# praateekmahajan/moving-mnist-vae

Hardware: AMD Instinct MI355X
Metric: frames/sec/GPU VAE train step, 20×64×64 batch; ELBO vs CPU ref (higher is better)
Workload: dtype bf16; 1 GPU; BASELINE configs[1]: 256 clips x 20 frames x 64x64 per GPU per step (=5120 frames), conv-VAE z=128, Gaussian NLL sigma=0.1 + KL (normal_vae_1_kl_0_mmd), Adam, random-init weights, Bernoulli(0.0521) q=2 labels; parallelism=dp1, rccl_ranks=1, grad_exchange=none, bn=per-rank batch statistics

## Files before the change

moving-mnist-vae_amd/csrc/conv_deep2.inc:

```
#include "kernels.hpp"
#include "tile_common.hpp"

namespace mmvae {

template <typename T, typename TO, int NPT, int CPT, bool ACC, bool LITE, bool F8 = false>
__device__ __forceinline__ void deep2_conv_body(const DeepArgs& a) {
  static_assert(!F8 || (sizeof(T) == 2 && !ACC), "fp8 MFMA: bf16 storage, forward convolutions");
  constexpr int VE = Elem<T>::kVec;
  constexpr int ES = sizeof(T);
  constexpr int TPX = NPT * 16;
  constexpr int kSV = 8;
  constexpr int G = CPT < (LITE ? 2 : 4) ? CPT : (LITE ? 2 : 4);
  constexpr int NB = LITE ? 2 : NPT >= 8 ? 3 : 4;
  constexpr int UPT = CPT / G;
  extern __shared__ __attribute__((aligned(16))) char smem[];
  const int t = threadIdx.x, nthr = blockDim.x, lane = t & 63, wv = __builtin_amdgcn_readfirstlane(t >> 6), gq = lane >> 4, r = lane & 15;
  const int c0 = (blockIdx.y * a.nw + wv) * 32;
  const int cin_vecs = a.Cin / VE;
  constexpr int LES = F8 ? 1 : ES;
  const int pitch = F8 ? a.Cin + 16 : a.Cin * ES + 32;
  const int npix_in = a.ipt * a.Hi * a.Wi;
  char* sPatch = smem;
  unsigned* sOpix = reinterpret_cast<unsigned*>(sPatch + (size_t)(npix_in + 1) * pitch);
  float* sStat = reinterpret_cast<float*>(sOpix + TPX) + wv * 64;
  unsigned short* sTab = reinterpret_cast<unsigned short*>(sOpix + TPX + 64 * a.nw);
  const T* __restrict__ X = reinterpret_cast<const T*>(a.x);
  TO* __restrict__ Y = reinterpret_cast<TO*>(a.y);
  const bool has_pro = a.pro_scale != nullptr, has_bias = a.bias != nullptr, has_stats = a.stats != nullptr;
  const float relu_lo = a.pro_relu ? 0.f : -__builtin_inff();
  const int HqWq = a.Hq * a.Wq;

  const int cv = t % cin_vecs, pix0 = t / cin_vecs, PS = nthr / cin_vecs;
  for (int p = t; p < TPX; p += nthr) {
    unsigned o = ~0u;
    int img = 0, hq = 0, wq = 0;
    const bool live = p < a.ipt * HqWq;
    if (live) {
      img = p / HqWq;
      const int rem = p - img * HqWq;
      hq = rem / a.Wq; wq = rem - hq * a.Wq;
      o = ((unsigned)img << 16) | ((unsigned)hq << 8) | (unsigned)wq;
    }
    sOpix[p] = o;
    const int hb = hq * a.SI, wb = wq * a.SI, ib = img * a.Hi;
#pragma unroll
    for (int tap = 0; tap < kMaxTaps; ++tap)
      if (tap < a.ntaps_all) {
        const int hi = hb + a.taps[tap].dh, wi = wb + a.taps[tap].dw;
        const bool in = live && hi >= 0 && hi < a.Hi && wi >= 0 && wi < a.Wi;
        sTab[tap * TPX + p] = (unsigned short)(in ? (ib + hi) * a.Wi + wi : npix_in);
      }
  }
  for (int i = t; i < pitch / 16; i += nthr) reinterpret_cast<Vec16*>(sPatch + (size_t)npix_in * pitch)[i] = Vec16{{0, 0, 0, 0}};
  sStat[lane] = 0.f;

  for (int tile = blockIdx.x; tile < a.ntiles; tile += gridDim.x) {
    const int n0 = tile * a.ipt;
    const int nimg = min(a.ipt, a.N - n0);
    __syncthreads();
    {
      const T* src = X + (long)n0 * a.Hi * a.Wi * a.Cin + cv * VE;
      const int nvalid = nimg * a.Hi * a.Wi;
      float psc[VE], psh[VE];
#pragma unroll
      for (int j = 0; j < VE; j += 4) {
        const float4 sc = has_pro ? *reinterpret_cast<const float4*>(a.pro_scale + cv * VE + j) : make_float4(1.f, 1.f, 1.f, 1.f);
        const float4 sh = has_pro ? *reinterpret_cast<const float4*>(a.pro_shift + cv * VE + j) : make_float4(0.f, 0.f, 0.f, 0.f);
        psc[j] = sc.x; psc[j + 1] = sc.y; psc[j + 2] = sc.z; psc[j + 3] = sc.w;
        psh[j] = sh.x; psh[j + 1] = sh.y; psh[j + 2] = sh.z; psh[j + 3] = sh.w;
      }
      for (int p0 = pix0; p0 < npix_in; p0 += kSV * PS) {
        Vec16 q[kSV];
#pragma unroll
        for (int k = 0; k < kSV; ++k) {
          const int p = p0 + k * PS;
          q[k] = Vec16{{0, 0, 0, 0}};
          if (p < nvalid) q[k] = *reinterpret_cast<const Vec16*>(src + (long)p * a.Cin);
        }
#pragma unroll
        for (int k = 0; k < kSV; ++k) {
          const int p = p0 + k * PS;
          if (p < npix_in) {
            if (has_pro && p < nvalid) {
              float f[VE];
              Elem<T>::unpack(q[k], f);
#pragma unroll
              for (int j = 0; j < VE; ++j) f[j] = fmaxf(f[j] * psc[j] + psh[j], relu_lo);
              q[k] = Elem<T>::pack(f);
            }
            if constexpr (F8) {
              float f[VE];
              Elem<T>::unpack(q[k], f);
              *reinterpret_cast<uint2*>(sPatch + (size_t)p * pitch + cv * 8) = pack8_fp8(f);
            } else {
              *reinterpret_cast<Vec16*>(sPatch + (size_t)p * pitch + cv * 16) = q[k];
            }
          }
        }
      }
    }
    __syncthreads();
    for (int ph = 0; ph < a.nphase; ++ph) {
      const DeepPhase P = a.phases[ph];
      const long rowbytes = (long)P.ntaps * a.Cin * LES;
      const int cstride = a.wfrag ? 1024 : 64;
      const char* wl0 = reinterpret_cast<const char*>(a.w) + P.w_off * LES +
                        (a.wfrag ? (long)c0 * rowbytes + lane * 16 : (long)(c0 + 8 * (r >> 2) + (r & 3)) * rowbytes + gq * 16);
      const char* wl1 = wl0 + (a.wfrag ? 16 : 4) * rowbytes;
      f32x4 acc[2][NPT];
#pragma unroll
      for (int m = 0; m < 2; ++m)
#pragma unroll
        for (int pt = 0; pt < NPT; ++pt) acc[m][pt] = (f32x4){0, 0, 0, 0};
      const int nunits = P.ntaps * UPT;
      auto load_unit = [&](Vec16 (&buf)[G][2], int unit) {
        const int jb = min(unit, nunits - 1) * G * cstride;
#pragma unroll
        for (int g = 0; g < G; ++g) {
          buf[g][0] = *reinterpret_cast<const Vec16*>(wl0 + jb + g * cstride);
          buf[g][1] = *reinterpret_cast<const Vec16*>(wl1 + jb + g * cstride);
        }
      };
      auto tap_pixels = [&](unsigned (&pb)[NPT], int tap) {
        const unsigned short* tb = sTab + (P.tap0 + tap) * TPX + r;
#pragma unroll
        for (int pt = 0; pt < NPT; ++pt) pb[pt] = __umul24((unsigned)tb[pt * 16], (unsigned)pitch) + gq * (F8 ? 8 : 16);
      };
      auto mul_unit = [&](const Vec16 (&buf)[G][2], const unsigned (&pb)[NPT], int cc0) {
#pragma unroll
        for (int g = 0; g < G; ++g) {
          if constexpr (F8) {
            long bl[NPT], bh[NPT];
#pragma unroll
            for (int pt = 0; pt < NPT; ++pt) {
              bl[pt] = *reinterpret_cast<const long*>(sPatch + pb[pt] + (cc0 + g) * 64);
              bh[pt] = *reinterpret_cast<const long*>(sPatch + pb[pt] + (cc0 + g) * 64 + 32);
            }
#pragma unroll
            for (int m = 0; m < 2; ++m) {
              const long al = (long)(((unsigned long)buf[g][m].w[1] << 32) | buf[g][m].w[0]);
              const long ah = (long)(((unsigned long)buf[g][m].w[3] << 32) | buf[g][m].w[2]);
#pragma unroll
              for (int pt = 0; pt < NPT; ++pt) {
                acc[m][pt] = __builtin_amdgcn_mfma_f32_16x16x32_fp8_fp8(al, bl[pt], acc[m][pt], 0, 0, 0);
                acc[m][pt] = __builtin_amdgcn_mfma_f32_16x16x32_fp8_fp8(ah, bh[pt], acc[m][pt], 0, 0, 0);
              }
            }
          } else {
            Vec16 bf[NPT];
#pragma unroll
            for (int pt = 0; pt < NPT; ++pt) bf[pt] = *reinterpret_cast<const Vec16*>(sPatch + pb[pt] + (cc0 + g) * 64);
#pragma unroll
            for (int pt = 0; pt < NPT; ++pt) {
              acc[0][pt] = mma_vec<T>(buf[g][0], bf[pt], acc[0][pt]);
              acc[1][pt] = mma_vec<T>(buf[g][1], bf[pt], acc[1][pt]);
            }
          }
        }
      };
      Vec16 buf[NB][G][2];
      unsigned pb[NPT];
#pragma unroll
      for (int b = 0; b < NB - 1; ++b) load_unit(buf[b], b);
      for (int u = 0; u < nunits; u += NB) {
#pragma unroll
        for (int b = 0; b < NB; ++b) {
          const int uu = u + b;
          load_unit(buf[(b + NB - 1) % NB], uu + NB - 1);
          __builtin_amdgcn_sched_barrier(0);
          if (uu < nunits) {
            if (UPT == 1 || (uu & (UPT - 1)) == 0) tap_pixels(pb, uu / UPT);
            mul_unit(buf[b], pb, (uu & (UPT - 1)) * G);
          }
          __builtin_amdgcn_sched_barrier(0);
        }
      }
      float bv[8], st1[8], st2[8];
#pragma unroll
      for (int j = 0; j < 8; ++j) {
        bv[j] = has_bias ? a.bias[c0 + 8 * gq + j] : 0.f;
        st1[j] = 0.f; st2[j] = 0.f;
      }
#pragma unroll
      for (int pt = 0; pt < NPT; ++pt) {
        const unsigned op = sOpix[pt * 16 + r];
        const int img = (int)(op >> 16), hq = (int)((op >> 8) & 255u), wq = (int)(op & 255u);
        if (op != ~0u && img < nimg && hq < P.Hq && wq < P.Wq) {
          const unsigned ob = ((((unsigned)(n0 + img) * a.Ho + (unsigned)(hq * a.SO + P.ph)) * a.Wo + (unsigned)(wq * a.SO + P.pw)) * (unsigned)a.Cout) +
                              (unsigned)(c0 + 8 * gq);
          float v[8];
#pragma unroll
          for (int j = 0; j < 8; ++j) v[j] = acc[j >> 2][pt][j & 3] + bv[j];
#pragma unroll
          for (int j = 0; j < 8; ++j) { st1[j] += v[j]; st2[j] += v[j] * v[j]; }
          dstore8<TO>(Y + ob, v, ACC);
        }
      }
      if (has_stats) {
#pragma unroll
        for (int j = 0; j < 8; ++j) { st1[j] = row16_sum(st1[j]); st2[j] = row16_sum(st2[j]); }
        if (r == 0) {
#pragma unroll
          for (int j = 0; j < 8; ++j) {
            sStat[8 * gq + j] += st1[j];
            sStat[32 + 8 * gq + j] += st2[j];
          }
        }
      }
    }
  }
  if (has_stats) {
    a.stats[(long)blockIdx.x * 2 * a.Cout + (long)(lane >> 5) * a.Cout + c0 + (lane & 31)] = sStat[lane];
  }
}

template <typename T, typename TO, int NPT, int CPT, bool ACC>
__global__ __launch_bounds__(512, 2) void deep2_conv_kernel(DeepArgs a) { deep2_conv_body<T, TO, NPT, CPT, ACC, false>(a); }
template <typename T, typename TO, int NPT, int CPT, bool ACC>
__global__ __launch_bounds__(512, 3) void deep2_conv_lite_kernel(DeepArgs a) { deep2_conv_body<T, TO, NPT, CPT, ACC, true>(a); }
template <typename T, typename TO, int NPT, int CPT, bool ACC>
__global__ __launch_bounds__(512, 2) void deep2_conv_f8_kernel(DeepArgs a) { deep2_conv_body<T, TO, NPT, CPT, false, false, true>(a); }
template <typename T, typename TO, int NPT, int CPT, bool ACC>
__global__ __launch_bounds__(512, 3) void deep2_conv_f8_lite_kernel(DeepArgs a) { deep2_conv_body<T, TO, NPT, CPT, false, true, true>(a); }

template <typename T, typename TO>
static int launch_deep2_t(const DeepArgs& a, int dt, int gx, hipStream_t s) {
  const size_t lds = deep2_conv_lds_bytes(a, dt);
  dim3 grid(gx, a.Cout / (32 * a.nw)), block(64 * a.nw);
#define MMVAE_D2K(K_, N_, C_, A_) do { \
    static bool attr_set = false; \
    if (!attr_set) { \
      const hipError_t e = hipFuncSetAttribute(reinterpret_cast<const void*>(&K_<T, TO, N_, C_, A_>), hipFuncAttributeMaxDynamicSharedMemorySize, 160 * 1024); \
      if (e != hipSuccess) { set_error("deep2_conv: hipFuncSetAttribute: %s", hipGetErrorString(e)); return MMVAE_ERR_HIP; } \
      attr_set = true; \
    } \
    hipLaunchKernelGGL((K_<T, TO, N_, C_, A_>), grid, block, lds, s, a); } while (0)
#define MMVAE_D2(N_, C_, A_) do { if (a.nw >= 4) MMVAE_D2K(deep2_conv_lite_kernel, N_, C_, A_); else MMVAE_D2K(deep2_conv_kernel, N_, C_, A_); } while (0)
#define MMVAE_D2C(N_, C_) do { if (a.accumulate) MMVAE_D2(N_, C_, true); else MMVAE_D2(N_, C_, false); } while (0)
#define MMVAE_D2N(N_) do { \
    constexpr int kC0 = sizeof(T) == 2 ? 1 : 2;       \
    if (cpt == kC0) MMVAE_D2C(N_, kC0); else if (cpt == 2 * kC0) MMVAE_D2C(N_, 2 * kC0); else if (cpt == 4 * kC0) MMVAE_D2C(N_, 4 * kC0); \
    else if (cpt == 8 * kC0) MMVAE_D2C(N_, 8 * kC0); \
    else { set_error("deep2_conv: Cin=%d unsupported", a.Cin); return MMVAE_ERR_UNSUPPORTED; } } while (0)
  const int cpt = 1 << a.cpt_log2;
  if (a.fp8) {
    if constexpr (sizeof(T) == 2 && sizeof(TO) == 2) {
      if (a.accumulate || !a.wfrag) { set_error("deep2_conv: fp8 needs fragment-major weights and no accumulate"); return MMVAE_ERR_UNSUPPORTED; }
#define MMVAE_D2F(N_, C_) do { if (a.nw >= 4 && N_ < 8) MMVAE_D2K(deep2_conv_f8_lite_kernel, N_, C_, false); else MMVAE_D2K(deep2_conv_f8_kernel, N_, C_, false); } while (0)
#define MMVAE_D2FN(N_) do { if (cpt == 1) MMVAE_D2F(N_, 1); else if (cpt == 2) MMVAE_D2F(N_, 2); else if (cpt == 4) MMVAE_D2F(N_, 4); \
      else { set_error("deep2_conv: fp8 Cin=%d unsupported", a.Cin); return MMVAE_ERR_UNSUPPORTED; } } while (0)
      if (a.npt == 8) MMVAE_D2FN(8); else if (a.npt == 4) MMVAE_D2FN(4); else if (a.npt == 2) MMVAE_D2FN(2);
      else { set_error("deep2_conv: npt=%d unsupported", a.npt); return MMVAE_ERR_UNSUPPORTED; }
#undef MMVAE_D2FN
#undef MMVAE_D2F
      const int rc8 = check_launch("deep2_conv_f8");
      return rc8 ? rc8 : gx;
    } else { set_error("deep2_conv: fp8 needs bf16 storage"); return MMVAE_ERR_UNSUPPORTED; }
  }
  if (a.npt == 8) MMVAE_D2N(8);
  else if (a.npt == 4) MMVAE_D2N(4);
  else if (a.npt == 2) MMVAE_D2N(2);
  else { set_error("deep2_conv: npt=%d unsupported", a.npt); return MMVAE_ERR_UNSUPPORTED; }
#undef MMVAE_D2N
#undef MMVAE_D2C
#undef MMVAE_D2
#undef MMVAE_D2K
  const int rc = check_launch("deep2_conv");
  return rc ? rc : gx;
}

#if DEEP_TU == 0
int launch_deep2_conv_f32(const DeepArgs& a, int gx, hipStream_t s) { return launch_deep2_t<float, float>(a, DT_F32, gx, s); }
#elif DEEP_TU == 1
int launch_deep2_conv_bf16(const DeepArgs& a, int gx, hipStream_t s) { return launch_deep2_t<bf16_t, bf16_t>(a, DT_BF16, gx, s); }
#else
int launch_deep2_conv_bf16_f32(const DeepArgs& a, int gx, hipStream_t s) { return launch_deep2_t<bf16_t, float>(a, DT_BF16, gx, s); }
#endif

}
```

moving-mnist-vae_amd/csrc/conv_gemm.hip:

```cpp
#include <stdlib.h>
#include <string.h>

#include <vector>

#include "kernels.hpp"

namespace mmvae {

constexpr int KV = 8;

__device__ __forceinline__ int lds_slot(int row, int kv) { return row * KV + (kv ^ ((row >> 1) & 7)); }

template <typename T> struct Mma;
template <> struct Mma<bf16_t> {
  __device__ static __forceinline__ f32x4 run(const Vec16& a, const Vec16& b, f32x4 c) {
    return __builtin_amdgcn_mfma_f32_16x16x32_bf16(__builtin_bit_cast(bf16x8, a), __builtin_bit_cast(bf16x8, b), c, 0, 0, 0);
  }
};
template <> struct Mma<float> {
  __device__ static __forceinline__ f32x4 run(const Vec16& a, const Vec16& b, f32x4 c) {
#pragma unroll
    for (int j = 0; j < 4; ++j)
      c = __builtin_amdgcn_mfma_f32_16x16x4f32(__uint_as_float(a.w[j]), __uint_as_float(b.w[j]), c, 0, 0, 0);
    return c;
// ... 287 lines not shown
  if (uni_ok && (Hq * a.SO != a.Ho || Wq * a.SO != a.Wo || (!a.y_planes && a.Cout % 16 != 0))) uni_ok = false;
  const size_t out_es = out_dt == DT_F32 ? 4 : dtype_size(dt);
  size_t lds = 0;
  int slots = 0;
  bool ok = false;
  TileGeom g1;
  const bool have1 = make_tile_geom(g1, a.N, Hq, Wq, a.Hi, a.Wi, a.SI, dh0, dw0, dh1 - dh0 + 1, dw1 - dw0 + 1, 128, 1);
  if (!have1) return 0;
  for (int sub = uni_ok ? max_sub : 1; sub >= 1 && !ok; sub >>= 1) {
    if (sub > 1 && Hq * Wq < 128 * sub) continue;
    if (!make_tile_geom(b.g, a.N, Hq, Wq, a.Hi, a.Wi, a.SI, dh0, dw0, dh1 - dh0 + 1, dw1 - dw0 + 1, 128, sub)) continue;
    if (sub > 1 && (b.g.tiles_per_img == 0 || b.g.qr * Wq != 128 * sub)) continue;
    if (sub > 1 && b.g.ntiles < 1024 && g1.ntiles >= 1024) continue;
    b.npt = 2 * sub;
    b.uni = (uni_ok && b.g.tiles_per_img > 0 && b.g.qr * Wq == 128 * sub) ? 1 : 0;
    if (sub > 1 && !b.uni) continue;
    b.out_wave_bytes = !b.uni ? 0 : (int)(a.y_planes ? (size_t)a.y_planes * b.npt * 16 * 4 : (size_t)b.npt * a.SO * ct16 * 4 * (16 * 4 * out_es + 16));
    b.out_wave_bytes = (b.out_wave_bytes + 15) & ~15;
    if (a.x2) {
      if (b.npt != 2) continue;
      b.x2_slots = (b.g.segs * b.g.qr * Wq * (a.Cin2 / VE) + 255) / 256;
      if (b.x2_slots > 4) continue;
    }
    lds = patch_conv_lds_bytes(b, dt);
    slots = patch_conv_slots(b, dt);
    ok = lds <= (sub > 1 ? 48 * 1024 : kV2MaxLds) && slots <= 12;
    if (!ok && b.uni && sub == 1) {
      b.uni = 0; b.out_wave_bytes = 0;
      lds = patch_conv_lds_bytes(b, dt);
      ok = lds <= kV2MaxLds && slots <= 12;
    }
    if (ok) { b.wq_shift = 0; while ((1 << b.wq_shift) < Wq) ++b.wq_shift; }
  }
  if (!ok) return 0;
  int occ = (int)((160 * 1024) / lds);
  const int occ_regs = slots <= 4 ? (ct16 == 1 ? 4 : (ct16 == 2 ? 3 : 2)) : ((slots <= 8 && ct16 == 1 && !a.x_planar) ? 3 : 2);
  if (occ > occ_regs) occ = occ_regs;
  if (occ < 1) occ = 1;
  int gx = 256 * occ;
  if (b.npt >= 4 && slots <= 4 && occ > occ_regs - 1 && occ > 1) occ = occ_regs - 1;
  gx = 256 * occ;
  if (gx > b.g.ntiles) gx = b.g.ntiles;
  if (gx > kGatherMaxGridX) gx = kGatherMaxGridX;
  if (gx >= 8) gx &= ~7;
  b.x_bytes = a.x_planar ? 0u : (unsigned)((long)a.N * a.Hi * a.Wi * a.Cin * (long)dtype_size(dt));
  if (a.x2) {
    if (ct16 > 2) return 0;
    patch_conv_x2_carve(b, dt);
    if (occ > 2 && ct16 == 1 && slots <= 4) { occ = occ_regs - 1 > 1 ? occ_regs - 1 : 1; gx = 256 * occ; if (gx > b.g.ntiles) gx = b.g.ntiles; if (gx > kGatherMaxGridX) gx = kGatherMaxGridX; if (gx >= 8) gx &= ~7; }
  }
  return launch_patch_conv(dt, out_dt, b, gx, s);
}

static size_t deep2_lds_for(int dt, int Cin, int Cout, int hw, int HiWi, int ntaps_all, int npt, int fp8 = 0) {
  DeepArgs b; memset(&b, 0, sizeof(b));
  b.fp8 = fp8;
  b.Cin = Cin; b.Hi = HiWi; b.Wi = 1; b.ipt = npt * 16 / hw; b.npt = npt; b.ntaps_all = ntaps_all; b.nw = Cout / 32 < 8 ? Cout / 32 : 8;
  return deep2_conv_lds_bytes(b, dt);
}
static bool deep2_shape_ok(int dt, int Cin, int Cout, int Hq, int Wq, int Hi, int Wi, int ntaps_all, int fp8) {
  if (fp8 && dt != DT_BF16) return false;
  const int ES = fp8 ? 1 : dt == DT_F32 ? 4 : 2;
  const int cpt = Cin * ES / 64;
  const int c0 = ES == 4 ? 2 : 1;
  if (Cin < (fp8 ? 64 : 32) || (Cin * ES) % 64 != 0 || (cpt != c0 && cpt != 2 * c0 && cpt != 4 * c0 && cpt != 8 * c0)) return false;
  if (Cout < 32 || Cout % 32 != 0 || (Cout > 256 && Cout % 256 != 0)) return false;
  if (Cin < 64 && Cout < 64) return false;
  const int hw = Hq * Wq;
  if (hw < 1 || hw > 128 || Hq > 255 || Wq > 255 || ntaps_all < 1 || ntaps_all > kMaxTaps) return false;
  const int npt_min = hw > 64 ? 8 : hw > 32 ? 4 : 2;
  if (fp8 && cpt > 4) return false;
  return deep2_lds_for(dt, Cin, Cout, hw, Hi * Wi, ntaps_all, npt_min, fp8) <= 150 * 1024;
}
static int try_deep2(int dt, int out_dt, const GatherArgs& a, hipStream_t s, bool dry = false) {
  if (a.x_planar || a.y_planes || a.x2) return 0;
  if (a.fp8 && (!a.wfrag || a.accumulate || dt != DT_BF16 || out_dt != DT_BF16)) return 0;
  int Hq = 0, Wq = 0, ntaps_all = 0;
  for (int p = 0; p < a.nphase; ++p) {
    const Phase& ph = a.phases[p];
    if (ph.ntaps <= 0) return 0;
    Hq = ph.Hq > Hq ? ph.Hq : Hq; Wq = ph.Wq > Wq ? ph.Wq : Wq;
    ntaps_all = ph.tap0 + ph.ntaps > ntaps_all ? ph.tap0 + ph.ntaps : ntaps_all;
  }
  if (!deep2_shape_ok(dt, a.Cin, a.Cout, Hq, Wq, a.Hi, a.Wi, ntaps_all, a.fp8)) return 0;
  if ((long)a.N * a.Ho * a.Wo * a.Cout >= (1L << 32)) return 0;
  const int ES = dt == DT_F32 ? 4 : 2, VE = 16 / ES;
  const int cpt = a.Cin * (a.fp8 ? 1 : ES) / 64;
  DeepArgs b; memset(&b, 0, sizeof(b));
  b.fp8 = a.fp8;
  b.x = a.x; b.w = a.w; b.y = a.y; b.pro_scale = a.pro_scale; b.pro_shift = a.pro_shift; b.pro_relu = a.pro_relu;
  b.bias = a.bias; b.stats = a.stats; b.accumulate = a.accumulate; b.wfrag = a.wfrag;
  b.N = a.N; b.Hi = a.Hi; b.Wi = a.Wi; b.Cin = a.Cin; b.Ho = a.Ho; b.Wo = a.Wo; b.Cout = a.Cout; b.SI = a.SI; b.SO = a.SO;
  b.nphase = a.nphase; b.Hq = Hq; b.Wq = Wq; b.ntaps_all = ntaps_all;
  for (int p = 0; p < a.nphase; ++p) {
    const Phase& ph = a.phases[p];
    b.phases[p] = DeepPhase{ph.ph, ph.pw, ph.Hq, ph.Wq, ph.ntaps, ph.tap0, ph.w_off};
  }
  for (int t = 0; t < kMaxTaps; ++t) b.taps[t] = a.taps[t];
  for (b.cpt_log2 = 0; (1 << b.cpt_log2) < cpt; ++b.cpt_log2) {}
  b.nw = a.Cout / 32 < 8 ? a.Cout / 32 : 8;
  if ((64 * b.nw) % (a.Cin / VE) != 0) return 0;
  const int gy = a.Cout / (32 * b.nw);
  const int hw = Hq * Wq;
  int best = 0;
  for (int pass = 0; pass < 2 && !best; ++pass)
    for (int npt = 8; npt >= 2 && !best; npt >>= 1) {
      if (hw > npt * 16) break;
      const size_t lds = deep2_lds_for(dt, a.Cin, a.Cout, hw, a.Hi * a.Wi, ntaps_all, npt, a.fp8);
      int ipt = npt * 16 / hw; if (ipt > a.N) ipt = a.N;
      const long ntiles = (a.N + ipt - 1) / ipt;
      if (pass == 0) {
        if (lds > 80 * 1024) continue;
        if (npt > 2 && ntiles * gy * b.nw < 256 * 4) continue;
      } else if (lds > 150 * 1024) continue;
      best = npt;
    }
  if (!best) return 0;
  if (dry) return 1;
  b.npt = best; b.ipt = best * 16 / hw;
  if (b.ipt > a.N) b.ipt = a.N;
  b.ntiles = (a.N + b.ipt - 1) / b.ipt;
  int gx = b.ntiles < kGatherMaxGridX ? b.ntiles : kGatherMaxGridX;
  return launch_deep2_conv(dt, out_dt, b, gx, s);
}

static int try_pos(int dt, int out_dt, const GatherArgs& a, hipStream_t s, bool dry = false) {
  if (dt != DT_BF16 || out_dt != DT_BF16 || !a.wfrag || a.fp8 || a.gup == 0) return 0;
  if (a.x_planar || a.y_planes || a.x2 || a.bias || a.Hi != a.Wi || a.Ho != a.Wo || a.Cout < 32 || a.Cout % 32 != 0) return 0;
  if (a.Cin < 8 || a.Cin % 8 != 0) return 0;
  const int up = a.gup == 2 ? 1 : 0;
  if (up && a.gs > 1 && a.gk < a.gs && !a.accumulate) return 0;
  if (a.Hi >= 8 && a.Cout < 128) return 0;
  if ((long)a.N * a.Ho * a.Wo * a.Cout >= (1L << 32)) return 0;
  PosArgs b; memset(&b, 0, sizeof(b));
  b.x = a.x; b.w = a.w; b.y = a.y; b.pro_scale = a.pro_scale; b.pro_shift = a.pro_shift; b.pro_relu = a.pro_relu;
  b.stats = a.stats; b.accumulate = a.accumulate; b.N = a.N; b.Cout = a.Cout;
  b.nw = a.Cout / 32 < 8 ? a.Cout / 32 : 8;
  if ((a.Cout / 32) % b.nw != 0 || (64 * b.nw) % (a.Cin / 8) != 0) return 0;
  return launch_pos_conv(a.gk, a.gs, a.gp, up, a.Hi, a.Ho, a.Cin, dry ? nullptr : &b, s);
}
bool gather_deep2_takes(int dt, int out_dt, const GatherArgs& a) { return try_deep2(dt, out_dt, a, nullptr, true) > 0; }
bool gather_pos_takes(int dt, int out_dt, const GatherArgs& a) { return try_pos(dt, out_dt, a, nullptr, true) > 0; }

static int launch_x2_separately(int dt, int out_dt, const GatherArgs& a, hipStream_t s) {
  GatherArgs b; memset(&b, 0, sizeof(b));
  int Hq = 0, Wq = 0;
  for (int p = 0; p < a.nphase; ++p) if (a.phases[p].ph == a.x2_ph && a.phases[p].pw == a.x2_pw) { Hq = a.phases[p].Hq; Wq = a.phases[p].Wq; }
  if (Hq <= 0) { set_error("gather_gemm: the second source's phase (%d,%d) is not part of the launch", a.x2_ph, a.x2_pw); return MMVAE_ERR_ARG; }
  b.x = a.x2; b.w = a.w2; b.y = a.y; b.accumulate = 1; b.wfrag = a.wfrag2;
  b.N = a.N; b.Hi = Hq; b.Wi = Wq; b.Cin = a.Cin2; b.Ho = a.Ho; b.Wo = a.Wo; b.Cout = a.Cout; b.SI = 1; b.SO = a.SO;
  b.nphase = 1; b.phases[0] = Phase{a.x2_ph, a.x2_pw, Hq, Wq, 1, 0, 0}; b.taps[0] = Tap{0, 0};
  b.gk = 1; b.gs = a.SO; b.gp = 0; b.gup = 2;
  return launch_gather_gemm(dt, out_dt, b, s);
}

int launch_gather_gemm(int dt, int out_dt, GatherArgs a, hipStream_t s) {
  const int VE = dt == DT_F32 ? 4 : 8;
  note_launch_bytes((double)a.N * ((double)a.Hi * a.Wi * (a.x_planar ? a.x_planes : a.Cin) * (a.x_planar == 1 ? 4 : dtype_size(dt)) +
                                   (double)a.Ho * a.Wo * (a.y_planes > 0 ? a.y_planes : a.Cout) * (a.y_planes > 0 ? 4 : dtype_size(out_dt)) +
                                   (a.x2 ? (double)a.phases[0].Hq * a.phases[0].Wq * a.Cin2 * dtype_size(dt) : 0.0)));
  if (a.fp8) {
    if (dt != DT_BF16 || out_dt != DT_BF16 || a.x2 || a.accumulate) { set_error("gather_gemm: fp8 needs the bf16 forward path"); return MMVAE_ERR_UNSUPPORTED; }
    a.cin_vecs = a.Cin / VE;
    const int rc2 = try_deep2(dt, out_dt, a, s);
    if (rc2 != 0) return rc2;
    if (a.wfrag) { set_error("gather_gemm: fragment-major fp8 weights (Cin=%d Cout=%d) need the deep2 kernel", a.Cin, a.Cout); return MMVAE_ERR_UNSUPPORTED; }
    set_error("gather_gemm: fp8 layer Cin=%d Cout=%d is not eligible for the deep-layer kernel", a.Cin, a.Cout); return MMVAE_ERR_UNSUPPORTED;
  }
  if (a.x2) {
    int rc = (!a.wfrag && !a.wfrag2) ? try_patch(dt, out_dt, a, s) : 0;
    if (rc != 0) return rc;
    GatherArgs m = a; m.x2 = nullptr; m.w2 = nullptr; m.Cin2 = 0; m.wfrag2 = 0;
// ... 424 lines not shown
```

moving-mnist-vae_amd/csrc/conv_wgrad.hip:

```cpp
#include <cstdlib>
#include "kernels.hpp"

namespace mmvae {

int launch_wgrad2_bf16(const Wgrad2Args& a, dim3 grid, int ta16, int tb16, int maxg, hipStream_t s);
int launch_wgrad2_f32(const Wgrad2Args& a, dim3 grid, int ta16, int tb16, int maxg, hipStream_t s);

int wgrad2_taps_per_block(int ta16, int tb16, int ntaps) {
  int mt = 12 / (ta16 * tb16); if (mt < 1) mt = 1; if (mt > 4) mt = 4;
  const int tg = ntaps >= 4 ? 4 * mt : mt;
  return tg < ntaps ? tg : ntaps;
}

size_t wgrad2_lds_bytes(const Wgrad2Args& a, int dt, int TA, int TB) {
  const size_t es = dtype_size(dt);
  const size_t stage = (size_t)a.g.TP * TA * es + (size_t)a.g.segs * a.g.PR * a.g.PW * TB * es + 32 * 4;
  const size_t acc1 = (size_t)TA * TB * 4;
  return stage > acc1 ? stage : acc1;
}

int wgrad2_patch_slots(const Wgrad2Args& a, int dt, int TB) {
  const int cvg = TB * (int)dtype_size(dt) / 16;
  const int nt = 64 * (a.nw > 0 ? a.nw : 4);
  const int per_round = nt / cvg;
// ... 75 lines not shown
  int lanes = 64;
  while (lanes > 8 && wsize / (4 * lanes) < 256) lanes >>= 1;
  const dim3 grid((unsigned)(wsize / (4 * lanes)));
  switch (lanes) {
    case 64: hipLaunchKernelGGL(wgrad_reduce_kernel<64>, grid, dim3(256), 0, s, a); break;
    case 32: hipLaunchKernelGGL(wgrad_reduce_kernel<32>, grid, dim3(256), 0, s, a); break;
    case 16: hipLaunchKernelGGL(wgrad_reduce_kernel<16>, grid, dim3(256), 0, s, a); break;
    default: hipLaunchKernelGGL(wgrad_reduce_kernel<8>, grid, dim3(256), 0, s, a); break;
  }
  return check_launch("wgrad_reduce");
}

int launch_patch_conv_f32(const PatchArgs& a, int gx, hipStream_t s);
int launch_patch_conv_bf16(const PatchArgs& a, int gx, hipStream_t s);
int launch_patch_conv_bf16_f32(const PatchArgs& a, int gx, hipStream_t s);

size_t patch_conv_lds_bytes(const PatchArgs& a, int dt) {
  const int VE = dt == DT_F32 ? 4 : 8;
  const int cin_vecs = a.Cin / VE;
  int ct16 = (a.Cout + 15) / 16; if (ct16 == 3) ct16 = 4;
  size_t b = (size_t)a.w_vecs * 16 + (size_t)a.g.segs * a.g.PR * a.g.PW * cin_vecs * 16 + (size_t)a.koff_total * 4 + (size_t)8 * ct16 * 16 * 4 +
             (a.uni ? (size_t)4 * a.out_wave_bytes : 0);
  b = (b + 15) & ~(size_t)15;
  if (a.x2) b += (size_t)ct16 * 16 * (a.kvp2 + 1) * 16 + ((size_t)a.g.segs * a.g.qr * a.g.Wq * (a.Cin2 / VE) + 8) * 16;
  return b;
}
void patch_conv_x2_carve(PatchArgs& a, int dt) {
  PatchArgs z = a; z.x2 = nullptr;
  const size_t base = patch_conv_lds_bytes(z, dt);
  int ct16 = (a.Cout + 15) / 16; if (ct16 == 3) ct16 = 4;
  a.w2_vec0 = (int)(base / 16);
  a.x2_vec0 = a.w2_vec0 + ct16 * 16 * (a.kvp2 + 1);
}

int patch_conv_slots(const PatchArgs& a, int dt) {
  const int VE = dt == DT_F32 ? 4 : 8;
  const int npatch = a.g.segs * a.g.PR * a.g.PW;
  const int per_round = a.x_planar ? 256 : 256 / (a.Cin / VE);
  return (npatch + per_round - 1) / per_round;
}

int launch_patch_conv(int dt, int out_dt, const PatchArgs& a, int gx, hipStream_t s) {
  if (dt == DT_F32) return launch_patch_conv_f32(a, gx, s);
  if (out_dt == DT_F32) return launch_patch_conv_bf16_f32(a, gx, s);
  return launch_patch_conv_bf16(a, gx, s);
}

int launch_deep2_conv_f32(const DeepArgs& a, int gx, hipStream_t s);
int launch_deep2_conv_bf16(const DeepArgs& a, int gx, hipStream_t s);
int launch_deep2_conv_bf16_f32(const DeepArgs& a, int gx, hipStream_t s);

size_t deep2_conv_lds_bytes(const DeepArgs& a, int dt) {
  const size_t pitch = a.fp8 ? (size_t)a.Cin + 16 : (size_t)a.Cin * dtype_size(dt) + 32;
  return (size_t)(a.ipt * a.Hi * a.Wi + 1) * pitch + (size_t)a.npt * 16 * 4 + (size_t)a.nw * 64 * 4 + (size_t)a.ntaps_all * a.npt * 16 * 2;
}

int launch_deep2_conv(int dt, int out_dt, const DeepArgs& a, int gx, hipStream_t s) {
  if (dt == DT_F32) return launch_deep2_conv_f32(a, gx, s);
  if (out_dt == DT_F32) return launch_deep2_conv_bf16_f32(a, gx, s);
  return launch_deep2_conv_bf16(a, gx, s);
}

}
```

moving-mnist-vae_amd/csrc/kernels.hpp:

```cpp
#pragma once
#include "common.hpp"

namespace mmvae {

enum DType : int { DT_F32 = 0, DT_BF16 = 1 };
inline size_t dtype_size(int dt) { return dt == DT_F32 ? 4 : 2; }

struct Tap { int dh, dw; };
constexpr int kMaxTaps = 25;
constexpr int kMaxPhases = 4;
struct Phase { int ph, pw, Hq, Wq, ntaps, tap0; long w_off;  };
struct GatherArgs {
  const void* x; const void* w; void* y;
  const float* pro_scale; const float* pro_shift; int pro_relu;
  const float* bias;
  float* stats;
  int accumulate;
  int N, Hi, Wi, Cin, Ho, Wo, Cout;
  int SI, SO;
  int nphase; Phase phases[kMaxPhases]; Tap taps[kMaxTaps];
  int cin_vecs;
  int x_planar, x_planes;
  int y_planes;
  const void* x2; const void* w2; int Cin2, x2_ph, x2_pw;
// ... 60 lines not shown
struct Wgrad2Args {
  const void* P; const void* G; float* dW;
  const float* proP_scale; const float* proP_shift; int proP_relu;
  const float* proG_scale; const float* proG_shift; int proG_relu;
  TileGeom g;
  int Ca, Cb, Cb_valid, Ca_valid, ksz, ntaps, TG;
  int sA, sB; int tap_off[25]; float scale;
  int P_planar, P_planes;
  int nw;
  int partial;
};
size_t wgrad2_lds_bytes(const Wgrad2Args& a, int dt, int TA, int TB);
int wgrad2_patch_slots(const Wgrad2Args& a, int dt, int TB);
int wgrad2_taps_per_block(int ta16, int tb16, int ntaps);
int launch_wgrad2(int dt, const Wgrad2Args& a, int gx, int tiles_ab, int zg, int ta16, int tb16, hipStream_t s);
size_t gather3_lds_bytes(const GatherArgs& a, int dt, int CT);
int launch_gather3(int dt, int out_dt, const GatherArgs& a, int gx, hipStream_t s);
struct WgradReduceArgs { const float* part; float* dW; int Ca, Cb, ntaps, nparts, Ca_valid, Cb_valid, sA, sB; int tap_off[25]; float scale; int exclusive;
                         long part_stride;  };
int launch_wgrad_reduce(WgradReduceArgs a, hipStream_t s);
constexpr size_t kWgradScratchBytes = 64u << 20;
struct PatchPhase { int ph, pw, Hq, Wq, ntaps, tap0; long w_off; int w_vec0, koff0; };
struct PatchArgs {
  const void* x; const void* w; void* y;
  const float* pro_scale; const float* pro_shift; int pro_relu;
  const float* bias; float* stats; int accumulate;
  int Cin, Cout, Ho, Wo, SO;
  TileGeom g;
  int nphase; PatchPhase phases[kMaxPhases]; Tap taps[kMaxTaps];
  int w_vecs, koff_total;
  int x_planar, x_planes, y_planes;
  int npt, wq_shift;
  int uni, out_wave_bytes;
  int phase_of[4];
  unsigned x_bytes;
  const void* x2; const void* w2; int Cin2, x2_phase, kvp2, w2_vec0, x2_vec0, x2_slots; unsigned x2_bytes;
};
size_t patch_conv_lds_bytes(const PatchArgs& a, int dt);
void patch_conv_x2_carve(PatchArgs& a, int dt);
int patch_conv_slots(const PatchArgs& a, int dt);
int launch_patch_conv(int dt, int out_dt, const PatchArgs& a, int gx, hipStream_t s);
struct DeepPhase { int ph, pw, Hq, Wq, ntaps, tap0; long w_off; };
struct DeepArgs {
  const void* x; const void* w; void* y;
  const float* pro_scale; const float* pro_shift; int pro_relu;
  const float* bias; float* stats; int accumulate;
  int N, Hi, Wi, Cin, Ho, Wo, Cout, SI, SO;
  int Hq, Wq;
  int nphase; DeepPhase phases[kMaxPhases]; Tap taps[kMaxTaps]; int ntaps_all;
  int ipt, ntiles;
  int ct16, npt;
  int fp8;
  int nw, cpt_log2;
  int wfrag;
};
size_t deep2_conv_lds_bytes(const DeepArgs& a, int dt);
int launch_deep2_conv(int dt, int out_dt, const DeepArgs& a, int gx, hipStream_t s);
struct PosArgs {
  const void* x; const void* w; void* y;
  const float* pro_scale; const float* pro_shift; int pro_relu;
  float* stats; int accumulate;
  int N, Cout;
  int nw;
  int ntiles;
};
int launch_pos_conv(int K, int S, int P, int up, int HI, int HO, int CIN, const PosArgs* a, hipStream_t s);

struct PackArgs {
  const float* src; void* dst; int cols, K, ntaps; int s_col, s_k; int tap_off[kMaxTaps]; float scale;
  int cols_valid, K_valid;
  int fp8;
  int frag;
};
int launch_pack(int dt, const PackArgs& a, hipStream_t s);
void pack_batch_begin();
int pack_batch_flush(int dt, hipStream_t s);

int launch_stem_im2col(int dt, const void* x, void* col, int N, int H, int W, int Ho, int Wo, hipStream_t s);

bool stem_bwd_fusable(int S);
bool conv3_stream_ok(int dt, int Cin, int Cout, int k, int s, int p, int Hin, int Win);
int launch_conv3_stream_bwd(int dt, const void* dy, const void* w_flipped, void* dx, const void* ym, const float* ms, const float* mb, float* sums,
                            int N, int H, hipStream_t s);
int launch_conv3_stream(int dt, int stride, const void* x, const void* w, const void* wsc, void* y, void* ysc, const float* pro_scale,
                        const float* pro_shift, int pro_relu, float* stats, float* stats_sc, int N, int Ho, hipStream_t s);
bool convT4_stream_ok(int dt, int Cin, int Cout, int k, int s, int p, int Hin, int Win);
int launch_convT4_stream(int dt, const void* x, const void* w_up, void* y, const float* pro_scale, const float* pro_shift, int pro_relu, float* stats,
                         int N, int Hin, hipStream_t s, int f8out = 0);
bool tail_fwd_stream_ok(int dt, int OC, int H, int W);
int launch_tail_fwd_stream(int dt, const void* y2, const float* s2, const float* b2, const void* ys, const float* ss, const float* bs, const float* w,
                           const float* bias, float* r_raw, float* stats, int N, int H, int W, hipStream_t s, int f8in = 0);
bool up5_tail_fwd_ok(int dt, int OC, int C, int Cin, int Hin, int Hout);
int launch_up5_tail_fwd(const void* y1, const float* p1s, const float* p1b, const void* w2_up, const void* xin, const float* pxs, const float* pxb,
                        const void* wu_up, const float* s2, const float* b2, const float* ss, const float* bs, const float* w, const float* bias,
                        float* r_raw, float* stats, int N, hipStream_t s);
bool stem_fwd_stream_ok(int dt, int S);
int launch_stem_fwd_stream(int dt, const void* x, const float* w, void* y, float* stats, int N, int S, hipStream_t s);
int stem_bwd_part_floats();
int launch_stem_gram(int dt, const void* x, float* scratch, long scratch_cap_floats, double* R, int N, int S, int Ho, int Wo, hipStream_t s);
int launch_stem_bwd(int dt, const void* g, const void* y0, const void* x, const float* ms, const float* mb, float* partials,
                    long partials_cap_floats, int N, int S, int Ho, int Wo, hipStream_t s);
bool stem_bwd_dg_ok(int dt, int S);
int launch_stem_bwd_dg(const void* dy1, const void* dys, const void* wd1, const void* wds, const void* y0, const void* x, const float* ms, const float* mb,
                       float* partials, long partials_cap_floats, int N, int S, int Ho, int Wo, hipStream_t s);
int launch_stem_bwd_finalize(const float* partials, int nparts, const double* R, const float* w, const float* global_sums, double count,
                             const float* gamma, const float* mean, const float* istd, float* dgamma, float* dbeta, float* dW, hipStream_t s);
// ... 118 lines not shown
```

Measured before the change: 847,300 frames/s.

## Split deep conv pixel tiles across extra waves for narrow-Cout layers

```diff
diff --git a/moving-mnist-vae_amd/csrc/conv_deep2.inc b/moving-mnist-vae_amd/csrc/conv_deep2.inc
--- a/moving-mnist-vae_amd/csrc/conv_deep2.inc
+++ b/moving-mnist-vae_amd/csrc/conv_deep2.inc
@@ -3,19 +3,24 @@
 
 namespace mmvae {
 
-template <typename T, typename TO, int NPT, int CPT, bool ACC, bool LITE, bool F8 = false>
+template <typename T, typename TO, int NPT, int CPT, bool ACC, bool LITE, bool F8 = false, int SPLIT = 1>
 __device__ __forceinline__ void deep2_conv_body(const DeepArgs& a) {
   static_assert(!F8 || (sizeof(T) == 2 && !ACC), "fp8 MFMA: bf16 storage, forward convolutions");
+  static_assert(SPLIT == 1 || (!LITE && !F8 && NPT / SPLIT >= 2), "split forms: the plain kernel, at least two column tiles per wave");
+  constexpr int NPW = NPT / SPLIT;
   constexpr int VE = Elem<T>::kVec;
   constexpr int ES = sizeof(T);
   constexpr int TPX = NPT * 16;
-  constexpr int kSV = 8;
-  constexpr int G = CPT < (LITE ? 2 : 4) ? CPT : (LITE ? 2 : 4);
-  constexpr int NB = LITE ? 2 : NPT >= 8 ? 3 : 4;
+  constexpr int kSV = (!LITE && !F8 && SPLIT == 1 && NPT == 8) ? 16 : 8;
+  constexpr int GMAX = (LITE || SPLIT > 1) ? 2 : 4;
+  constexpr int G = CPT < GMAX ? CPT : GMAX;
+  constexpr int NB = (LITE || (SPLIT == 2 && G == 2)) ? 2 : NPT >= 8 ? 3 : 4;
   constexpr int UPT = CPT / G;
   extern __shared__ __attribute__((aligned(16))) char smem[];
   const int t = threadIdx.x, nthr = blockDim.x, lane = t & 63, wv = __builtin_amdgcn_readfirstlane(t >> 6), gq = lane >> 4, r = lane & 15;
-  const int c0 = (blockIdx.y * a.nw + wv) * 32;
+  const int cg = SPLIT == 1 ? wv : wv % a.nw;
+  const int pt0 = SPLIT == 1 ? 0 : (wv / a.nw) * NPW;
+  const int c0 = (blockIdx.y * a.nw + cg) * 32;
   const int cin_vecs = a.Cin / VE;
   constexpr int LES = F8 ? 1 : ES;
   const int pitch = F8 ? a.Cin + 16 : a.Cin * ES + 32;
@@ -23,14 +28,14 @@
   char* sPatch = smem;
   unsigned* sOpix = reinterpret_cast<unsigned*>(sPatch + (size_t)(npix_in + 1) * pitch);
   float* sStat = reinterpret_cast<float*>(sOpix + TPX) + wv * 64;
-  unsigned short* sTab = reinterpret_cast<unsigned short*>(sOpix + TPX + 64 * a.nw);
+  unsigned short* sTab = reinterpret_cast<unsigned short*>(sOpix + TPX + 64 * a.nw * SPLIT);
   const T* __restrict__ X = reinterpret_cast<const T*>(a.x);
   TO* __restrict__ Y = reinterpret_cast<TO*>(a.y);
   const bool has_pro = a.pro_scale != nullptr, has_bias = a.bias != nullptr, has_stats = a.stats != nullptr;
   const float relu_lo = a.pro_relu ? 0.f : -__builtin_inff();
   const int HqWq = a.Hq * a.Wq;
 
-  const int cv = t % cin_vecs, pix0 = t / cin_vecs, PS = nthr / cin_vecs;
+  const int cv = t % cin_vecs, pix0 = t / cin_vecs, pstep = nthr / cin_vecs;
   for (int p = t; p < TPX; p += nthr) {
     unsigned o = ~0u;
     int img = 0, hq = 0, wq = 0;
@@ -69,17 +74,17 @@
         psc[j] = sc.x; psc[j + 1] = sc.y; psc[j + 2] = sc.z; psc[j + 3] = sc.w;
         psh[j] = sh.x; psh[j + 1] = sh.y; psh[j + 2] = sh.z; psh[j + 3] = sh.w;
       }
-      for (int p0 = pix0; p0 < npix_in; p0 += kSV * PS) {
+      for (int p0 = pix0; p0 < npix_in; p0 += kSV * pstep) {
         Vec16 q[kSV];
 #pragma unroll
         for (int k = 0; k < kSV; ++k) {
-          const int p = p0 + k * PS;
+          const int p = p0 + k * pstep;
           q[k] = Vec16{{0, 0, 0, 0}};
           if (p < nvalid) q[k] = *reinterpret_cast<const Vec16*>(src + (long)p * a.Cin);
         }
 #pragma unroll
         for (int k = 0; k < kSV; ++k) {
-          const int p = p0 + k * PS;
+          const int p = p0 + k * pstep;
           if (p < npix_in) {
             if (has_pro && p < nvalid) {
               float f[VE];
@@ -107,11 +112,11 @@
       const char* wl0 = reinterpret_cast<const char*>(a.w) + P.w_off * LES +
                         (a.wfrag ? (long)c0 * rowbytes + lane * 16 : (long)(c0 + 8 * (r >> 2) + (r & 3)) * rowbytes + gq * 16);
       const char* wl1 = wl0 + (a.wfrag ? 16 : 4) * rowbytes;
-      f32x4 acc[2][NPT];
+      f32x4 acc[2][NPW];
 #pragma unroll
       for (int m = 0; m < 2; ++m)
 #pragma unroll
-        for (int pt = 0; pt < NPT; ++pt) acc[m][pt] = (f32x4){0, 0, 0, 0};
+        for (int pt = 0; pt < NPW; ++pt) acc[m][pt] = (f32x4){0, 0, 0, 0};
       const int nunits = P.ntaps * UPT;
       auto load_unit = [&](Vec16 (&buf)[G][2], int unit) {
         const int jb = min(unit, nunits - 1) * G * cstride;
@@ -121,18 +126,18 @@
           buf[g][1] = *reinterpret_cast<const Vec16*>(wl1 + jb + g * cstride);
         }
       };
-      auto tap_pixels = [&](unsigned (&pb)[NPT], int tap) {
-        const unsigned short* tb = sTab + (P.tap0 + tap) * TPX + r;
-#pragma unroll
-        for (int pt = 0; pt < NPT; ++pt) pb[pt] = __umul24((unsigned)tb[pt * 16], (unsigned)pitch) + gq * (F8 ? 8 : 16);
+      auto tap_pixels = [&](unsigned (&pb)[NPW], int tap) {
+        const unsigned short* tb = sTab + (P.tap0 + tap) * TPX + pt0 * 16 + r;
+#pragma unroll
+        for (int pt = 0; pt < NPW; ++pt) pb[pt] = __umul24((unsigned)tb[pt * 16], (unsigned)pitch) + gq * (F8 ? 8 : 16);
       };
-      auto mul_unit = [&](const Vec16 (&buf)[G][2], const unsigned (&pb)[NPT], int cc0) {
+      auto mul_unit = [&](const Vec16 (&buf)[G][2], const unsigned (&pb)[NPW], int cc0) {
 #pragma unroll
         for (int g = 0; g < G; ++g) {
           if constexpr (F8) {
-            long bl[NPT], bh[NPT];
-#pragma unroll
-            for (int pt = 0; pt < NPT; ++pt) {
+            long bl[NPW], bh[NPW];
+#pragma unroll
+            for (int pt = 0; pt < NPW; ++pt) {
               bl[pt] = *reinterpret_cast<const long*>(sPatch + pb[pt] + (cc0 + g) * 64);
               bh[pt] = *reinterpret_cast<const long*>(sPatch + pb[pt] + (cc0 + g) * 64 + 32);
             }
@@ -141,17 +146,17 @@
               const long al = (long)(((unsigned long)buf[g][m].w[1] << 32) | buf[g][m].w[0]);
               const long ah = (long)(((unsigned long)buf[g][m].w[3] << 32) | buf[g][m].w[2]);
 #pragma unroll
-              for (int pt = 0; pt < NPT; ++pt) {
+              for (int pt = 0; pt < NPW; ++pt) {
                 acc[m][pt] = __builtin_amdgcn_mfma_f32_16x16x32_fp8_fp8(al, bl[pt], acc[m][pt], 0, 0, 0);
                 acc[m][pt] = __builtin_amdgcn_mfma_f32_16x16x32_fp8_fp8(ah, bh[pt], acc[m][pt], 0, 0, 0);
               }
             }
           } else {
-            Vec16 bf[NPT];
-#pragma unroll
-            for (int pt = 0; pt < NPT; ++pt) bf[pt] = *reinterpret_cast<const Vec16*>(sPatch + pb[pt] + (cc0 + g) * 64);
-#pragma unroll
-            for (int pt = 0; pt < NPT; ++pt) {
+            Vec16 bf[NPW];
+#pragma unroll
+            for (int pt = 0; pt < NPW; ++pt) bf[pt] = *reinterpret_cast<const Vec16*>(sPatch + pb[pt] + (cc0 + g) * 64);
+#pragma unroll
+            for (int pt = 0; pt < NPW; ++pt) {
               acc[0][pt] = mma_vec<T>(buf[g][0], bf[pt], acc[0][pt]);
               acc[1][pt] = mma_vec<T>(buf[g][1], bf[pt], acc[1][pt]);
             }
@@ -159,7 +164,7 @@
         }
       };
       Vec16 buf[NB][G][2];
-      unsigned pb[NPT];
+      unsigned pb[NPW];
 #pragma unroll
       for (int b = 0; b < NB - 1; ++b) load_unit(buf[b], b);
       for (int u = 0; u < nunits; u += NB) {
@@ -182,8 +187,8 @@
         st1[j] = 0.f; st2[j] = 0.f;
       }
 #pragma unroll
-      for (int pt = 0; pt < NPT; ++pt) {
-        const unsigned op = sOpix[pt * 16 + r];
+      for (int pt = 0; pt < NPW; ++pt) {
+        const unsigned op = sOpix[(pt0 + pt) * 16 + r];
         const int img = (int)(op >> 16), hq = (int)((op >> 8) & 255u), wq = (int)(op & 255u);
         if (op != ~0u && img < nimg && hq < P.Hq && wq < P.Wq) {
           const unsigned ob = ((((unsigned)(n0 + img) * a.Ho + (unsigned)(hq * a.SO + P.ph)) * a.Wo + (unsigned)(wq * a.SO + P.pw)) * (unsigned)a.Cout) +
@@ -210,7 +215,16 @@
     }
   }
   if (has_stats) {
-    a.stats[(long)blockIdx.x * 2 * a.Cout + (long)(lane >> 5) * a.Cout + c0 + (lane & 31)] = sStat[lane];
+    float v = sStat[lane];
+    if constexpr (SPLIT > 1) {
+      __syncthreads();
+      const float* row = reinterpret_cast<const float*>(sOpix + TPX) + cg * 64 + lane;
+      v = row[0];
+#pragma unroll
+      for (int k = 1; k < SPLIT; ++k) v += row[k * a.nw * 64];
+      if (pt0 != 0) return;
+    }
+    a.stats[(long)blockIdx.x * 2 * a.Cout + (long)(lane >> 5) * a.Cout + c0 + (lane & 31)] = v;
   }
 }
 
@@ -218,6 +232,10 @@
 __global__ __launch_bounds__(512, 2) void deep2_conv_kernel(DeepArgs a) { deep2_conv_body<T, TO, NPT, CPT, ACC, false>(a); }
 template <typename T, typename TO, int NPT, int CPT, bool ACC>
 __global__ __launch_bounds__(512, 3) void deep2_conv_lite_kernel(DeepArgs a) { deep2_conv_body<T, TO, NPT, CPT, ACC, true>(a); }
+template <typename T, typename TO, int NPT, int CPT, bool ACC>
+__global__ __launch_bounds__(256, 4) void deep2_conv_split2_kernel(DeepArgs a) { deep2_conv_body<T, TO, NPT, CPT, ACC, false, false, 2>(a); }
+template <typename T, typename TO, int NPT, int CPT, bool ACC>
+__global__ __launch_bounds__(256, 3) void deep2_conv_split4_kernel(DeepArgs a) { deep2_conv_body<T, TO, NPT, CPT, ACC, false, false, 4>(a); }
 template <typename T, typename TO, int NPT, int CPT, bool ACC>
 __global__ __launch_bounds__(512, 2) void deep2_conv_f8_kernel(DeepArgs a) { deep2_conv_body<T, TO, NPT, CPT, false, false, true>(a); }
 template <typename T, typename TO, int NPT, int CPT, bool ACC>
@@ -226,7 +244,8 @@
 template <typename T, typename TO>
 static int launch_deep2_t(const DeepArgs& a, int dt, int gx, hipStream_t s) {
   const size_t lds = deep2_conv_lds_bytes(a, dt);
-  dim3 grid(gx, a.Cout / (32 * a.nw)), block(64 * a.nw);
+  const int ps = a.ps > 1 ? a.ps : 1;
+  dim3 grid(gx, a.Cout / (32 * a.nw)), block(64 * a.nw * ps);
 #define MMVAE_D2K(K_, N_, C_, A_) do { \
     static bool attr_set = false; \
     if (!attr_set) { \
@@ -235,7 +254,13 @@
       attr_set = true; \
     } \
     hipLaunchKernelGGL((K_<T, TO, N_, C_, A_>), grid, block, lds, s, a); } while (0)
-#define MMVAE_D2(N_, C_, A_) do { if (a.nw >= 4) MMVAE_D2K(deep2_conv_lite_kernel, N_, C_, A_); else MMVAE_D2K(deep2_conv_kernel, N_, C_, A_); } while (0)
+#define MMVAE_D2(N_, C_, A_) do { \
+    if (ps > 1) { \
+      if constexpr (N_ >= 4) { if (ps == 2) { MMVAE_D2K(deep2_conv_split2_kernel, N_, C_, A_); break; } } \
+      if constexpr (N_ >= 8) { if (ps == 4) { MMVAE_D2K(deep2_conv_split4_kernel, N_, C_, A_); break; } } \
+      set_error("deep2_conv: split %d of npt=%d nw=%d unsupported", ps, a.npt, a.nw); return MMVAE_ERR_UNSUPPORTED; \
+    } \
+    if (a.nw >= 4) MMVAE_D2K(deep2_conv_lite_kernel, N_, C_, A_); else MMVAE_D2K(deep2_conv_kernel, N_, C_, A_); } while (0)
 #define MMVAE_D2C(N_, C_) do { if (a.accumulate) MMVAE_D2(N_, C_, true); else MMVAE_D2(N_, C_, false); } while (0)
 #define MMVAE_D2N(N_) do { \
     constexpr int kC0 = sizeof(T) == 2 ? 1 : 2;       \
@@ -243,6 +268,7 @@
     else if (cpt == 8 * kC0) MMVAE_D2C(N_, 8 * kC0); \
     else { set_error("deep2_conv: Cin=%d unsupported", a.Cin); return MMVAE_ERR_UNSUPPORTED; } } while (0)
   const int cpt = 1 << a.cpt_log2;
+  if (ps > 1 && (a.fp8 || a.nw * ps != 4)) { set_error("deep2_conv: split %d needs 4-wave blocks of the bf16 / f32 forms (nw=%d fp8=%d)", ps, a.nw, a.fp8); return MMVAE_ERR_UNSUPPORTED; }
   if (a.fp8) {
     if constexpr (sizeof(T) == 2 && sizeof(TO) == 2) {
       if (a.accumulate || !a.wfrag) { set_error("deep2_conv: fp8 needs fragment-major weights and no accumulate"); return MMVAE_ERR_UNSUPPORTED; }
diff --git a/moving-mnist-vae_amd/csrc/conv_gemm.hip b/moving-mnist-vae_amd/csrc/conv_gemm.hip
--- a/moving-mnist-vae_amd/csrc/conv_gemm.hip
+++ b/moving-mnist-vae_amd/csrc/conv_gemm.hip
@@ -363,10 +363,15 @@
   return launch_patch_conv(dt, out_dt, b, gx, s);
 }
 
+static int deep2_split_for(int nw, int npt, int fp8, int Cin, bool has_stats) {
+  const int ps = nw == 1 ? 4 : nw == 2 ? 2 : 1;
+  return !fp8 && !has_stats && Cin <= 64 && npt / ps >= 2 ? ps : 1;
+}
 static size_t deep2_lds_for(int dt, int Cin, int Cout, int hw, int HiWi, int ntaps_all, int npt, int fp8 = 0) {
   DeepArgs b; memset(&b, 0, sizeof(b));
   b.fp8 = fp8;
   b.Cin = Cin; b.Hi = HiWi; b.Wi = 1; b.ipt = npt * 16 / hw; b.npt = npt; b.ntaps_all = ntaps_all; b.nw = Cout / 32 < 8 ? Cout / 32 : 8;
+  b.ps = deep2_split_for(b.nw, npt, fp8, Cin, false);
   return deep2_conv_lds_bytes(b, dt);
 }
 static bool deep2_shape_ok(int dt, int Cin, int Cout, int Hq, int Wq, int Hi, int Wi, int ntaps_all, int fp8) {
@@ -429,6 +434,7 @@
   if (!best) return 0;
   if (dry) return 1;
   b.npt = best; b.ipt = best * 16 / hw;
+  b.ps = deep2_split_for(b.nw, best, a.fp8, a.Cin, a.stats != nullptr);
   if (b.ipt > a.N) b.ipt = a.N;
   b.ntiles = (a.N + b.ipt - 1) / b.ipt;
   int gx = b.ntiles < kGatherMaxGridX ? b.ntiles : kGatherMaxGridX;
diff --git a/moving-mnist-vae_amd/csrc/conv_wgrad.hip b/moving-mnist-vae_amd/csrc/conv_wgrad.hip
--- a/moving-mnist-vae_amd/csrc/conv_wgrad.hip
+++ b/moving-mnist-vae_amd/csrc/conv_wgrad.hip
@@ -151,7 +151,7 @@
 
 size_t deep2_conv_lds_bytes(const DeepArgs& a, int dt) {
   const size_t pitch = a.fp8 ? (size_t)a.Cin + 16 : (size_t)a.Cin * dtype_size(dt) + 32;
-  return (size_t)(a.ipt * a.Hi * a.Wi + 1) * pitch + (size_t)a.npt * 16 * 4 + (size_t)a.nw * 64 * 4 + (size_t)a.ntaps_all * a.npt * 16 * 2;
+  return (size_t)(a.ipt * a.Hi * a.Wi + 1) * pitch + (size_t)a.npt * 16 * 4 + (size_t)a.nw * (a.ps > 1 ? a.ps : 1) * 64 * 4 + (size_t)a.ntaps_all * a.npt * 16 * 2;
 }
 
 int launch_deep2_conv(int dt, int out_dt, const DeepArgs& a, int gx, hipStream_t s) {
diff --git a/moving-mnist-vae_amd/csrc/kernels.hpp b/moving-mnist-vae_amd/csrc/kernels.hpp
--- a/moving-mnist-vae_amd/csrc/kernels.hpp
+++ b/moving-mnist-vae_amd/csrc/kernels.hpp
@@ -136,6 +136,7 @@
   int ct16, npt;
   int fp8;
   int nw, cpt_log2;
+  int ps;
   int wfrag;
 };
 size_t deep2_conv_lds_bytes(const DeepArgs& a, int dt);
```

Result: no change. 848,700 frames/s, median of 6 (+0.2%).
